# microsoft/UniSpeech

Hardware: NVIDIA H100
Metric: audio-sec/sec fwd+bwd (higher is better)
Workload: dtype bf16

## Files before the change

unispeech_b200/csrc/gemm.cu:

```cuda
#include <stdarg.h>
#include <stdlib.h>

#include <algorithm>
#include <mutex>

#include "../../include/unispeech_b200.h"
#include "common.h"
#include "gemm.cuh"

namespace b200 {

long long g_launch_count = 0;
static thread_local char g_err[512] = "";
char* last_error_buf() { return g_err; }
void set_last_error(const char* fmt, ...) {
  va_list ap;
  va_start(ap, fmt);
  vsnprintf(g_err, sizeof(g_err), fmt, ap);
  va_end(ap);
}
bool pdl_enabled() {
  static int v = -1;
  if (v < 0) {
    const char* e = getenv("B200S_PDL");
// ... 162 lines not shown

static int gemm_rows_impl(const void* a, long long a_bs, long long a_rs, int rows, int batches, int K, const void* w, int N,
                          void* out, long long out_bs, long long out_ld, const b200s_epilogue* epi, const int* m_valid,
                          b200s_stream stream) {
  B200_CHECK_ARG(a && w && out, "gemm_rows: null pointer");
  B200_CHECK_ARG(rows > 0 && batches > 0 && K > 0 && N > 0, "gemm_rows: bad sizes");
  B200_CHECK_ARG(K % 64 == 0, "gemm_rows: K=%d must be a multiple of 64", K);
  B200_CHECK_ARG(N % 8 == 0, "gemm_rows: N=%d must be a multiple of 8", N);
  if (check_epilogue(epi)) return -1;
  cudaStream_t st = static_cast<cudaStream_t>(stream);

  CUtensorMap ta, tb;
  ViewSpec va{a, {K, rows, batches, 1}, {a_rs, batches > 1 ? a_bs : 0, 0}, {64, 128, 1, 1}};
  if (batches == 1) va.strides[1] = 0;
  if (make_tmap(&ta, va)) return -3;

  GemmParams p;
  memset(&p, 0, sizeof(p));
  fill_epilogue(p, epi);
  p.out = {out, out_bs, out_ld};
  p.m_rows = rows;
  p.m_tile_stride = 128;
  p.m_tile_valid = 128;
  p.m_tiles_per_batch = ceil_div(rows, 128);
  p.m_tiles = p.m_tiles_per_batch * batches;
  p.n_total = N;
  p.k_blocks = K / 64;
  p.m_valid = m_valid;

  if (N >= 256 && m_valid == nullptr) {
    ViewSpec vb{w, {K, N, 1, 1}, {K, 0, 0}, {64, 256, 1, 1}};
    if (make_tmap(&tb, vb)) return -3;
    static std::once_flag once;
    static cudaError_t attr_err = cudaSuccess;
    std::call_once(once, [] {
      attr_err = cudaFuncSetAttribute(gemm_ws_kernel, cudaFuncAttributeMaxDynamicSharedMemorySize, WsCfg::kSmemBytes);
    });
    B200_CHECK_CUDA(attr_err);
    const int tiles = p.m_tiles * ceil_div(N, 256);
    B200_CHECK_CUDA(launch_pdl(gemm_ws_kernel, dim3(std::min(tiles, sm_count())), dim3(WsCfg::kThreads), WsCfg::kSmemBytes, st,
                               ta, tb, p));
    B200_CHECK_LAUNCH();
    return 0;
  }

  const int block_n = (N >= 128) ? 128 : 64;
  ViewSpec vb{w, {K, N, 1, 1}, {K, 0, 0}, {64, block_n, 1, 1}};
  if (make_tmap(&tb, vb)) return -3;

  p.n_out_stride = block_n;
  p.n_tile_valid = block_n;
  p.k_blocks_per_batch = 0;
  p.k_blocks_per_split = p.k_blocks;
  p.ca[0][4] = 1; p.ca[1][1] = 1; p.ca[2][2] = 1;
  p.cb[0][4] = 1; p.cb[1][3] = block_n;
  dim3 grid(ceil_div(N, block_n), p.m_tiles_per_batch * batches, 1);
  B200_CHECK_ARG(grid.y <= 65535, "gemm_rows: too many M tiles (%u)", grid.y);
  return block_n == 128 ? launch_gemm<128, false, false>(ta, tb, p, grid, st)
                        : launch_gemm<64, false, false>(ta, tb, p, grid, st);
}

int b200s_reserve_sms(int sms) {
  B200_CHECK_ARG(sms >= 0 && sms < sm_count(), "reserve_sms: %d out of range", sms);
  return 0;
}

int b200s_gemm_rows(const void* a, long long a_bs, long long a_rs, int rows, int batches, int K, const void* w, int N,
                    void* out, long long out_bs, long long out_ld, const b200s_epilogue* epi, b200s_stream stream) {
  return gemm_rows_impl(a, a_bs, a_rs, rows, batches, K, w, N, out, out_bs, out_ld, epi, nullptr, stream);
}

int b200s_gemm_rows_ragged(const void* a, long long a_bs, long long a_rs, int rows, int batches, int K, const void* w, int N,
                           void* out, long long out_bs, long long out_ld, const b200s_epilogue* epi, const int* m_valid,
                           b200s_stream stream) {
  return gemm_rows_impl(a, a_bs, a_rs, rows, batches, K, w, N, out, out_bs, out_ld, epi, m_valid, stream);
}

static int gemm_wgrad_impl(const void* y, long long y_bs, long long y_rs, const void* x, long long x_bs, long long x_rs,
                           int rows, int batches, int N, int K, float* dw, long long dw_ld, const int* k_valid,
                           b200s_stream stream) {
  B200_CHECK_ARG(y && x && dw, "gemm_wgrad: null pointer");
  B200_CHECK_ARG(rows > 0 && batches > 0 && K > 0 && N > 0, "gemm_wgrad: bad sizes");
  B200_CHECK_ARG(N % 8 == 0 && K % 8 == 0, "gemm_wgrad: N=%d, K=%d must be multiples of 8", N, K);
  const int block_n = (K >= 128) ? 128 : 64;

  CUtensorMap ta, tb;
  ViewSpec va{y, {N, rows, batches, 1}, {y_rs, batches > 1 ? y_bs : 0, 0}, {64, 64, 1, 1}};
  if (make_tmap(&ta, va)) return -3;
  ViewSpec vb{x, {K, rows, batches, 1}, {x_rs, batches > 1 ? x_bs : 0, 0}, {64, 64, 1, 1}};
  if (make_tmap(&tb, vb)) return -3;

  GemmParams p;
  memset(&p, 0, sizeof(p));
  p.m_rows = N;
  p.m_tile_stride = 128;
  p.m_tile_valid = 128;
  p.m_tiles_per_batch = ceil_div(N, 128);
  p.n_total = K;
  p.n_out_stride = block_n;
  p.n_tile_valid = block_n;
  p.k_blocks_per_batch = ceil_div(rows, 64);
  p.k_blocks = p.k_blocks_per_batch * batches;
  const int tiles = p.m_tiles_per_batch * ceil_div(K, block_n);
  int splits = ceil_div(2 * sm_count(), tiles);
  if (splits > p.k_blocks) splits = p.k_blocks;
  if (splits < 1) splits = 1;
  p.k_blocks_per_split = ceil_div(p.k_blocks, splits);
  splits = ceil_div(p.k_blocks, p.k_blocks_per_split);
  p.ca[0][1] = 1; p.ca[0][7] = 1; p.ca[1][4] = 1; p.ca[2][5] = 1;
  p.cb[0][3] = block_n; p.cb[0][7] = 1; p.cb[1][4] = 1; p.cb[2][5] = 1;
  p.flags = EPI_OUT_F32 | EPI_ATOMIC;
  fill_epilogue(p, nullptr);
  p.out = {dw, 0, dw_ld};
  p.k_valid = k_valid;
  dim3 grid(ceil_div(K, block_n), p.m_tiles_per_batch, splits);
  cudaStream_t st = static_cast<cudaStream_t>(stream);
  return block_n == 128 ? launch_gemm<128, true, true>(ta, tb, p, grid, st)
                        : launch_gemm<64, true, true>(ta, tb, p, grid, st);
}

int b200s_gemm_wgrad(const void* y, long long y_bs, long long y_rs, const void* x, long long x_bs, long long x_rs,
                     int rows, int batches, int N, int K, float* dw, long long dw_ld, b200s_stream stream) {
  return gemm_wgrad_impl(y, y_bs, y_rs, x, x_bs, x_rs, rows, batches, N, K, dw, dw_ld, nullptr, stream);
}

int b200s_gemm_wgrad_ragged(const void* y, long long y_bs, long long y_rs, const void* x, long long x_bs, long long x_rs,
                            int rows, int batches, int N, int K, float* dw, long long dw_ld, const int* k_valid,
                            b200s_stream stream) {
  return gemm_wgrad_impl(y, y_bs, y_rs, x, x_bs, x_rs, rows, batches, N, K, dw, dw_ld, k_valid, stream);
}

int b200s_posconv_gemm(const void* xpad, long long xpad_bs, int T, int B, int D, int G, int taps, const void* wp,
                       void* out, long long out_bs, long long out_ld, const b200s_epilogue* epi,
                       b200s_stream stream) {
  B200_CHECK_ARG(xpad && wp && out, "posconv_gemm: null pointer");
  B200_CHECK_ARG(D % G == 0, "posconv_gemm: D %% G != 0");
  const int Cg = D / G;
  B200_CHECK_ARG(Cg <= 64 && Cg % 8 == 0, "posconv_gemm: channels per group %d must be <=64 and a multiple of 8", Cg);
  B200_CHECK_ARG(D % 8 == 0, "posconv_gemm: D must be a multiple of 8");
  B200_CHECK_ARG(taps >= 1, "posconv_gemm: taps=%d must be positive", taps);
  if (check_epilogue(epi)) return -1;

  CUtensorMap ta, tb;
  ViewSpec vb{wp, {taps * 64LL, G * 64LL, 1, 1}, {taps * 64LL, 0, 0}, {64, 64, 1, 1}};
  if (make_tmap(&tb, vb)) return -3;

  GemmParams p;
  memset(&p, 0, sizeof(p));
  p.m_rows = T;
  p.m_tile_stride = 128;
  p.m_tile_valid = 128;
  p.m_tiles_per_batch = ceil_div(T, 128);
  p.n_total = D;
  p.n_out_stride = Cg;
  p.n_tile_valid = Cg;
  p.k_blocks = taps;
  p.k_blocks_per_batch = 0;
  p.k_blocks_per_split = taps;
  p.flags = 0;
  fill_epilogue(p, epi);
  p.out = {out, out_bs, out_ld};
  dim3 grid(G, p.m_tiles_per_batch * B, 1);
  cudaStream_t st = static_cast<cudaStream_t>(stream);

  if (taps <= 129) {
    ViewSpec vw{xpad, {D, T + taps - 1, B, 1}, {D, B > 1 ? xpad_bs : 0, 0}, {64, 256, 1, 1}};
    if (make_tmap(&ta, vw)) return -3;
    static std::once_flag once;
    static cudaError_t attr_err = cudaSuccess;
    std::call_once(once, [] {
      attr_err = cudaFuncSetAttribute(posconv_window_kernel, cudaFuncAttributeMaxDynamicSharedMemorySize,
                                      PosconvCfg::kSmemBytes);
    });
    B200_CHECK_CUDA(attr_err);
    B200_CHECK_CUDA(launch_pdl(posconv_window_kernel, grid, dim3(PosconvCfg::kThreads), PosconvCfg::kSmemBytes, st, ta, tb, p,
                               taps, Cg));
    B200_CHECK_LAUNCH();
    return 0;
  }
  ViewSpec va{xpad, {D, taps, T, B}, {D, D, xpad_bs}, {64, 1, 128, 1}};
  if (make_tmap(&ta, va)) return -3;
  p.ca[0][3] = Cg; p.ca[1][6] = 1; p.ca[2][1] = 1; p.ca[3][2] = 1;
  p.cb[0][4] = 1; p.cb[1][3] = 64;
  return launch_gemm<64, false, false>(ta, tb, p, grid, st);
}

int b200s_posconv_wgrad(const void* dy, long long dy_bs, long long dy_rs, const void* xpad, long long xpad_bs, int T,
                        int B, int D, int G, int taps, float* dwp, b200s_stream stream) {
  B200_CHECK_ARG(dy && xpad && dwp, "posconv_wgrad: null pointer");
  B200_CHECK_ARG(D % G == 0, "posconv_wgrad: D %% G != 0");
  const int Cg = D / G;
  B200_CHECK_ARG(Cg <= 64 && Cg % 8 == 0, "posconv_wgrad: channels per group %d must be <=64 and a multiple of 8", Cg);

  CUtensorMap ta, tb;
  ViewSpec va{dy, {D, T, B, 1}, {dy_rs, B > 1 ? dy_bs : 0, 0}, {64, 64, 1, 1}};
  if (make_tmap(&ta, va)) return -3;
  ViewSpec vb{xpad, {D, taps, T, B}, {D, D, xpad_bs}, {64, 1, 64, 1}};
  if (make_tmap(&tb, vb)) return -3;

  GemmParams p;
  memset(&p, 0, sizeof(p));
// ... 21 lines not shown
```

unispeech_b200/csrc/gemm.cuh:

```cuda
#pragma once
#include "ptx.cuh"

namespace b200 {

struct EpiTensor {
  void* p;
  long long bs;
  long long ld;
};

enum : int {
  EPI_GELU = 1,
  EPI_DGELU = 2,
  EPI_OUT_F32 = 4,
  EPI_ATOMIC = 8,
  EPI_COLSUM = 16,
  EPI_ACCUM = 32,
  EPI_GELU_STORE_GRAD = 64,
  EPI_AUX_IS_GRAD = 128,
};

constexpr int kCoordVars = 8;

struct GemmParams {
// ... 51 lines not shown
  e.out_bf = static_cast<__nv_bfloat16*>(p.out.p) + mb * p.out.bs + row * p.out.ld;
  e.out_f32 = static_cast<float*>(p.out.p) + mb * p.out.bs + row * p.out.ld;
  e.out2 = p.out2.p ? static_cast<__nv_bfloat16*>(p.out2.p) + mb * p.out2.bs + row * p.out2.ld : nullptr;
  e.aux = p.aux.p ? static_cast<const __nv_bfloat16*>(p.aux.p) + mb * p.aux.bs + row * p.aux.ld : nullptr;
  e.res1 = p.res1.p ? static_cast<const __nv_bfloat16*>(p.res1.p) + mb * p.res1.bs + row * p.res1.ld : nullptr;
  e.res2 = p.res2.p ? static_cast<const __nv_bfloat16*>(p.res2.p) + mb * p.res2.bs + row * p.res2.ld : nullptr;
  return e;
}
__device__ __forceinline__ void add_bf16x8(float* a8, const __nv_bfloat16* src) {
  const uint4 w = *reinterpret_cast<const uint4*>(src);
  const uint32_t wu[4] = {w.x, w.y, w.z, w.w};
#pragma unroll
  for (int j = 0; j < 4; ++j) {
    const float2 f = unpack_bf16x2(wu[j]);
    a8[2 * j] += f.x;
    a8[2 * j + 1] += f.y;
  }
}
__device__ __forceinline__ uint4 pack_bf16x8(const float* a8) {
  uint4 w;
  w.x = pack_bf16x2(a8[0], a8[1]); w.y = pack_bf16x2(a8[2], a8[3]);
  w.z = pack_bf16x2(a8[4], a8[5]); w.w = pack_bf16x2(a8[6], a8[7]);
  return w;
}

__device__ __forceinline__ void epilogue_chunk32(const GemmParams& p, const EpiRow& e, const float* src, int c0, int n_valid,
                                                 int col_base, bool row_ok, int lane) {
  const int flags = p.flags;
  float acc[32];
#pragma unroll
  for (int j = 0; j < 8; ++j) {
    const float4 v = reinterpret_cast<const float4*>(src)[j];
    acc[4 * j] = v.x; acc[4 * j + 1] = v.y; acc[4 * j + 2] = v.z; acc[4 * j + 3] = v.w;
  }
  const bool full = (c0 + 32 <= n_valid);
  if (p.bias != nullptr) {
    const float* bp = p.bias + col_base + c0;
    if (full) {
#pragma unroll
      for (int j = 0; j < 8; ++j) {
        const float4 b4 = __ldg(reinterpret_cast<const float4*>(bp) + j);
        acc[4 * j] += b4.x; acc[4 * j + 1] += b4.y; acc[4 * j + 2] += b4.z; acc[4 * j + 3] += b4.w;
      }
    } else {
#pragma unroll
      for (int j = 0; j < 32; ++j)
        if (c0 + j < n_valid) acc[j] += __ldg(bp + j);
    }
  }
  if (row_ok) {
    const int col0 = col_base + c0;
#pragma unroll
    for (int g = 0; g < 4; ++g) {
      if (!full && (c0 + g * 8 >= n_valid)) break;
      const int col = col0 + g * 8;
      float* a8 = acc + g * 8;
      if (flags & EPI_GELU) {
        if (flags & EPI_GELU_STORE_GRAD) {
          float g8[8];
#pragma unroll
          for (int j = 0; j < 8; ++j) a8[j] = gelu_with_grad_f(a8[j], g8[j]);
          if (e.out2 != nullptr) *reinterpret_cast<uint4*>(e.out2 + col) = pack_bf16x8(g8);
        } else {
          if (e.out2 != nullptr) *reinterpret_cast<uint4*>(e.out2 + col) = pack_bf16x8(a8);
#pragma unroll
          for (int j = 0; j < 8; ++j) a8[j] = gelu_f(a8[j]);
        }
      }
      if (flags & EPI_DGELU) {
        const uint4 w = *reinterpret_cast<const uint4*>(e.aux + col);
        const uint32_t wu[4] = {w.x, w.y, w.z, w.w};
#pragma unroll
        for (int j = 0; j < 4; ++j) {
          const float2 f = unpack_bf16x2(wu[j]);
          a8[2 * j] *= (flags & EPI_AUX_IS_GRAD) ? f.x : gelu_grad_f(f.x);
          a8[2 * j + 1] *= (flags & EPI_AUX_IS_GRAD) ? f.y : gelu_grad_f(f.y);
        }
      }
      if (e.res1 != nullptr) add_bf16x8(a8, e.res1 + col);
      if (e.res2 != nullptr) add_bf16x8(a8, e.res2 + col);
      if (flags & EPI_OUT_F32) {
        float* o = e.out_f32 + col;
        if (flags & EPI_ATOMIC) {
          asm volatile("red.global.add.v4.f32 [%0], {%1, %2, %3, %4};" ::"l"(o), "f"(a8[0]), "f"(a8[1]), "f"(a8[2]), "f"(a8[3])
                       : "memory");
          asm volatile("red.global.add.v4.f32 [%0], {%1, %2, %3, %4};" ::"l"(o + 4), "f"(a8[4]), "f"(a8[5]), "f"(a8[6]),
                       "f"(a8[7])
                       : "memory");
        } else if (flags & EPI_ACCUM) {
          float4 o0 = *reinterpret_cast<float4*>(o), o1 = *reinterpret_cast<float4*>(o + 4);
          o0.x += a8[0]; o0.y += a8[1]; o0.z += a8[2]; o0.w += a8[3];
          o1.x += a8[4]; o1.y += a8[5]; o1.z += a8[6]; o1.w += a8[7];
          *reinterpret_cast<float4*>(o) = o0;
          *reinterpret_cast<float4*>(o + 4) = o1;
        } else {
          *reinterpret_cast<float4*>(o) = make_float4(a8[0], a8[1], a8[2], a8[3]);
          *reinterpret_cast<float4*>(o + 4) = make_float4(a8[4], a8[5], a8[6], a8[7]);
        }
      } else {
        *reinterpret_cast<uint4*>(e.out_bf + col) = pack_bf16x8(a8);
      }
    }
  }
  if (flags & EPI_COLSUM) {
    float cv[32];
#pragma unroll
    for (int j = 0; j < 32; ++j) {
      float t = row_ok ? acc[j] : 0.0f;
      if (!(flags & EPI_OUT_F32)) t = __bfloat162float(__float2bfloat16_rn(t));
      cv[j] = t;
    }
    const float csum = warp_colsum32(cv, lane);
    if ((c0 + lane) < n_valid) atomicAdd(p.colsum + col_base + c0 + lane, csum);
  }
}


template <int N, bool TA, bool TB>
__device__ __forceinline__ void wgmma_tile(float* acc, uint64_t da, uint64_t db, uint32_t scale_d) {
  if constexpr (N == 64) wgmma_m64n64k16<TA ? 1 : 0, TB ? 1 : 0>(acc, da, db, scale_d);
  else wgmma_m64n128k16<TA ? 1 : 0, TB ? 1 : 0>(acc, da, db, scale_d);
}

template <int BLOCK_N>
__device__ __forceinline__ void gemm_consumer_tail(const GemmParams& p, const float* acc, float* acc_s, int mb, int m0,
                                                   int col_base, int n_valid, int m_valid) {
  constexpr int kPitch = BLOCK_N + 8;
  const int ew = threadIdx.x >> 5, lane = threadIdx.x & 31;
  named_bar_sync(1, 256);
  acc_to_smem<BLOCK_N>(acc, acc_s, kPitch, 64 * (ew >> 2));
  named_bar_sync(1, 256);
  const int r = (ew & 3) * 32 + lane;
  const EpiRow erow = make_epi_row(p, mb, static_cast<long long>(m0) + r);
#pragma unroll 1
  for (int c0 = (ew >> 2) * (BLOCK_N / 2); c0 < ((ew >> 2) + 1) * (BLOCK_N / 2); c0 += 32) {
    if (c0 >= n_valid) break;
    epilogue_chunk32(p, erow, acc_s + r * kPitch + c0, c0, n_valid, col_base, r < m_valid, lane);
  }
}

__device__ __forceinline__ void zero_dead_tile(const GemmParams& p, int mb, int m0, int col_base, int n_valid) {
  const int rows = min(p.m_tile_valid, p.m_rows - m0), c8 = n_valid / 8;
  for (int i = threadIdx.x; i < rows * c8; i += blockDim.x) {
    const long long row = static_cast<long long>(m0) + i / c8;
    const int col = col_base + (i % c8) * 8;
    *reinterpret_cast<uint4*>(static_cast<__nv_bfloat16*>(p.out.p) + mb * p.out.bs + row * p.out.ld + col) = make_uint4(0u, 0u, 0u, 0u);
    if (p.out2.p != nullptr)
      *reinterpret_cast<uint4*>(static_cast<__nv_bfloat16*>(p.out2.p) + mb * p.out2.bs + row * p.out2.ld + col) = make_uint4(0u, 0u, 0u, 0u);
  }
}

template <int BLOCK_N, bool A_MN, bool B_MN>
__global__ void __launch_bounds__(288, 2) gemm_bf16_kernel(const __grid_constant__ CUtensorMap tmA,
                                                           const __grid_constant__ CUtensorMap tmB,
                                                           const __grid_constant__ GemmParams p) {
  pdl_launch_dependents();
  using Cfg = GemmCfg<BLOCK_N>;
  constexpr int kStages = Cfg::kStages;

  const int warp = threadIdx.x >> 5;
  const int lane = threadIdx.x & 31;
  const int n_tile = blockIdx.x;
  const int mb = blockIdx.y / p.m_tiles_per_batch;
  const int m0 = (blockIdx.y % p.m_tiles_per_batch) * p.m_tile_stride;
  const int kb_begin = blockIdx.z * p.k_blocks_per_split;
  const int kb_end = min(kb_begin + p.k_blocks_per_split, p.k_blocks);
  if (kb_begin >= kb_end) return;
  const int col_base = n_tile * p.n_out_stride;
  const int n_valid = min(p.n_tile_valid, p.n_total - col_base);

  extern __shared__ uint8_t smem_raw[];
// ... 42 lines not shown
          v[5] = 0;
          v[4] = kb * 64;
        }
        v[6] = kb;
        uint8_t* sa = smem + s * Cfg::kStageBytes;
        uint8_t* sb = sa + Cfg::kABytes;
        mbar_expect_tx(&full_bar[s], Cfg::kStageBytes);
        if constexpr (!A_MN) {
          v[7] = 0;
          tma_load_4d(sa, &tmA, &full_bar[s], coord_dot(p.ca[0], v), coord_dot(p.ca[1], v), coord_dot(p.ca[2], v),
                      coord_dot(p.ca[3], v));
        } else {
#pragma unroll
          for (int i = 0; i < 2; ++i) {
            v[7] = 64 * i;
            tma_load_4d(sa + i * 8192, &tmA, &full_bar[s], coord_dot(p.ca[0], v), coord_dot(p.ca[1], v),
                        coord_dot(p.ca[2], v), coord_dot(p.ca[3], v));
          }
        }
        if constexpr (!B_MN) {
          v[7] = 0;
          tma_load_4d(sb, &tmB, &full_bar[s], coord_dot(p.cb[0], v), coord_dot(p.cb[1], v), coord_dot(p.cb[2], v),
                      coord_dot(p.cb[3], v));
        } else {
#pragma unroll
          for (int i = 0; i < BLOCK_N / 64; ++i) {
            v[7] = 64 * i;
            tma_load_4d(sb + i * 8192, &tmB, &full_bar[s], coord_dot(p.cb[0], v), coord_dot(p.cb[1], v),
                        coord_dot(p.cb[2], v), coord_dot(p.cb[3], v));
          }
        }
      }
    }
  } else {
    const int c = warp >> 2;
    float acc[BLOCK_N / 2];
    int it = 0;
    for (int kb = kb_begin; kb < kb_end; ++kb) {
      if (!kb_live(kb)) continue;
      const int s = it % kStages;
      mbar_wait(&full_bar[s], (it / kStages) & 1);
      const uint32_t sa = smem_u32(smem + s * Cfg::kStageBytes) + c * 8192;
      const uint32_t sb = smem_u32(smem + s * Cfg::kStageBytes + Cfg::kABytes);
      wgmma_fence();
#pragma unroll
      for (int k = 0; k < 4; ++k) {
        const uint64_t da = A_MN ? make_smem_desc_sw128(sa + k * 2048, 8192, 1024) : make_smem_desc_sw128(sa + k * 32, 16, 1024);
        const uint64_t db = B_MN ? make_smem_desc_sw128(sb + k * 2048, 8192, 1024) : make_smem_desc_sw128(sb + k * 32, 16, 1024);
        wgmma_tile<BLOCK_N, A_MN, B_MN>(acc, da, db, (it > 0 || k > 0) ? 1u : 0u);
      }
      wgmma_commit();
      wgmma_wait<1>();
      if (it > 0 && lane == 0) mbar_arrive(&empty_bar[(it - 1) % kStages]);
      ++it;
    }
    wgmma_wait<0>();
    if (it == 0) {
#pragma unroll
      for (int i = 0; i < BLOCK_N / 2; ++i) acc[i] = 0.f;
    }
    gemm_consumer_tail<BLOCK_N>(p, acc, reinterpret_cast<float*>(smem), mb, m0, col_base, n_valid,
                                min(p.m_tile_valid, p.m_rows - m0));
  }
}

struct WsCfg {
  static constexpr int kStages = 3;
  static constexpr int kABytes = 128 * 128;
  static constexpr int kBBytes = 256 * 128;
  static constexpr int kStageBytes = kABytes + kBBytes;
  static constexpr int kEpiBytes = 64 * 64 * 4;
  static constexpr int kPfBytes = 3 * 8 * 128 * 8;
  static constexpr int kSmemBytes = kStages * kStageBytes + 2 * kEpiBytes + 2 * kPfBytes + 1024;
  static constexpr int kThreads = 384;
  static_assert(kSmemBytes + 1024 <= 232448, "one CTA per SM");
};

__device__ __forceinline__ void add_bf16x4(float* v, uint2 w) {
  const float2 f0 = unpack_bf16x2(w.x), f1 = unpack_bf16x2(w.y);
  v[0] += f0.x; v[1] += f0.y; v[2] += f1.x; v[3] += f1.y;
}
__device__ __forceinline__ uint2 pack_bf16x4(const float* v) { return make_uint2(pack_bf16x2(v[0], v[1]), pack_bf16x2(v[2], v[3])); }

__global__ void __launch_bounds__(384, 1) gemm_ws_kernel(const __grid_constant__ CUtensorMap tmA,
                                                         const __grid_constant__ CUtensorMap tmB,
                                                         const __grid_constant__ GemmParams p) {
  pdl_launch_dependents();
  using Cfg = WsCfg;
  constexpr int kStages = Cfg::kStages;
  const int wg = threadIdx.x >> 7;
  const int lane = threadIdx.x & 31;
  const int n_tiles = (p.n_total + 255) / 256;
  const int num_tiles = p.m_tiles * n_tiles;

  extern __shared__ uint8_t smem_raw[];
  uint8_t* smem = smem_raw + ((1024u - (smem_u32(smem_raw) & 1023u)) & 1023u);
  __shared__ uint64_t full_bar[kStages];
  __shared__ uint64_t empty_bar[kStages];

  if (threadIdx.x == 0) {
    tma_prefetch_desc(&tmA);
    tma_prefetch_desc(&tmB);
#pragma unroll
    for (int s = 0; s < kStages; ++s) {
      mbar_init(&full_bar[s], 1);
      mbar_init(&empty_bar[s], 8);
    }
    fence_mbar_init();
  }
  __syncthreads();
  pdl_wait();

  if (wg == 0) {
    setmaxnreg_dec<40>();
    if (threadIdx.x == 0) {
      int it = 0;
      for (int tile = blockIdx.x; tile < num_tiles; tile += gridDim.x) {
        const int mt = tile / n_tiles, n_tile = tile - mt * n_tiles;
        const int mb = mt / p.m_tiles_per_batch, m0 = (mt - mb * p.m_tiles_per_batch) * 128;
        for (int kb = 0; kb < p.k_blocks; ++kb, ++it) {
          const int s = it % kStages;
          mbar_wait(&empty_bar[s], ((it / kStages) & 1) ^ 1);
          uint8_t* sa = smem + s * Cfg::kStageBytes;
          mbar_expect_tx(&full_bar[s], Cfg::kStageBytes);
          tma_load_4d(sa, &tmA, &full_bar[s], kb * 64, m0, mb, 0);
          tma_load_4d(sa + Cfg::kABytes, &tmB, &full_bar[s], kb * 64, n_tile * 256, 0, 0);
        }
      }
    }
    return;
  }

  setmaxnreg_inc<232>();
  const int c = wg - 1;
  const int t = threadIdx.x & 127, w = t >> 5;
  float* stage = reinterpret_cast<float*>(smem + kStages * Cfg::kStageBytes + c * Cfg::kEpiBytes);
  uint2* pf = reinterpret_cast<uint2*>(smem + kStages * Cfg::kStageBytes + 2 * Cfg::kEpiBytes + c * Cfg::kPfBytes);
  const int cq = 4 * (lane & 15);
  const EpiTensor* const pf_src[3] = {&p.aux, &p.res1, &p.res2};
  float acc[128];
  int it = 0;
  for (int tile = blockIdx.x; tile < p.m_tiles * n_tiles; tile += gridDim.x) {
    const int mt = tile / n_tiles, n_tile = tile - mt * n_tiles;
    const int mb = mt / p.m_tiles_per_batch, m0 = (mt - mb * p.m_tiles_per_batch) * 128;
    const int col_base = n_tile * 256;
    const int n_valid = min(256, p.n_total - col_base);
    const int rows_here = min(128, p.m_rows - m0) - 64 * c;
    auto prefetch = [&](int j) {
      const int cl = 64 * j + cq;
      if (cl < n_valid) {
#pragma unroll
        for (int q = 0; q < 3; ++q) {
          const EpiTensor& e = *pf_src[q];
          if (e.p == nullptr) continue;
#pragma unroll
          for (int i = 0; i < 8; ++i) {
            const int r = 16 * w + 2 * i + (lane >> 4);
            if (r < rows_here)
              cp_async_8(pf + (q * 8 + i) * 128 + t, static_cast<const __nv_bfloat16*>(e.p) + mb * e.bs +
                                                         (static_cast<long long>(m0) + 64 * c + r) * e.ld + col_base + cl);
          }
        }
      }
      cp_async_commit();
    };
    prefetch(0);
    for (int kb = 0; kb < p.k_blocks; ++kb, ++it) {
      const int s = it % kStages;
      mbar_wait(&full_bar[s], (it / kStages) & 1);
      const uint32_t sa = smem_u32(smem + s * Cfg::kStageBytes) + c * 8192;
      const uint32_t sb = smem_u32(smem + s * Cfg::kStageBytes + Cfg::kABytes);
      wgmma_fence();
#pragma unroll
      for (int k = 0; k < 4; ++k)
        wgmma_m64n256k16<0, 0>(acc, make_smem_desc_sw128(sa + k * 32, 16, 1024), make_smem_desc_sw128(sb + k * 32, 16, 1024),
                               (kb > 0 || k > 0) ? 1u : 0u);
      wgmma_commit();
      wgmma_wait<1>();
      if (kb > 0 && lane == 0) mbar_arrive(&empty_bar[(it - 1) % kStages]);
    }
    wgmma_wait<0>();
    if (lane == 0) mbar_arrive(&empty_bar[(it - 1) % kStages]);

    const int flags = p.flags;
#pragma unroll
    for (int j = 0; j < 4; ++j) {
      if (64 * j >= n_valid) break;
      named_bar_sync(1 + c, 128);
#pragma unroll
      for (int i = 32 * j; i < 32 * j + 32; i += 2) {
        const int r = 16 * w + (lane >> 2) + 8 * ((i >> 1) & 1);
        const int cc = 8 * ((i >> 2) - 8 * j) + 2 * (lane & 3);
        *reinterpret_cast<float2*>(stage + r * 64 + (cc ^ ((r & 3) << 3))) = make_float2(acc[i], acc[i + 1]);
      }
      const int cl = 64 * j + cq;
      const bool col_ok = cl < n_valid;
      const int col = col_base + cl;
      named_bar_sync(1 + c, 128);
      float4 b4 = make_float4(0.f, 0.f, 0.f, 0.f);
      if (p.bias != nullptr && col_ok) b4 = __ldg(reinterpret_cast<const float4*>(p.bias + col));
      float cs[4] = {0.f, 0.f, 0.f, 0.f};
      cp_async_wait_all();
#pragma unroll 4
      for (int i = 0; i < 8; ++i) {
        const int r = 16 * w + 2 * i + (lane >> 4);
        const float4 v4 = *reinterpret_cast<const float4*>(stage + r * 64 + (cq ^ ((r & 3) << 3)));
        if (!col_ok || r >= rows_here) continue;
        float v[4] = {v4.x + b4.x, v4.y + b4.y, v4.z + b4.z, v4.w + b4.w};
        const long long row = static_cast<long long>(m0) + 64 * c + r;
        if (flags & EPI_GELU) {
          __nv_bfloat16* o2 =
              p.out2.p ? static_cast<__nv_bfloat16*>(p.out2.p) + mb * p.out2.bs + row * p.out2.ld + col : nullptr;
          if (flags & EPI_GELU_STORE_GRAD) {
            float g[4];
#pragma unroll
            for (int k = 0; k < 4; ++k) v[k] = gelu_with_grad_f(v[k], g[k]);
            if (o2 != nullptr) *reinterpret_cast<uint2*>(o2) = pack_bf16x4(g);
          } else {
            if (o2 != nullptr) *reinterpret_cast<uint2*>(o2) = pack_bf16x4(v);
#pragma unroll
            for (int k = 0; k < 4; ++k) v[k] = gelu_f(v[k]);
          }
        }
        if (flags & EPI_DGELU) {
          const uint2 a = pf[(0 * 8 + i) * 128 + t];
          const float2 f0 = unpack_bf16x2(a.x), f1 = unpack_bf16x2(a.y);
          const float f[4] = {f0.x, f0.y, f1.x, f1.y};
#pragma unroll
          for (int k = 0; k < 4; ++k) v[k] *= (flags & EPI_AUX_IS_GRAD) ? f[k] : gelu_grad_f(f[k]);
        }
        if (p.res1.p != nullptr) add_bf16x4(v, pf[(1 * 8 + i) * 128 + t]);
        if (p.res2.p != nullptr) add_bf16x4(v, pf[(2 * 8 + i) * 128 + t]);
        *reinterpret_cast<uint2*>(static_cast<__nv_bfloat16*>(p.out.p) + mb * p.out.bs + row * p.out.ld + col) = pack_bf16x4(v);
        if (flags & EPI_COLSUM) {
#pragma unroll
          for (int k = 0; k < 4; ++k) cs[k] += __bfloat162float(__float2bfloat16_rn(v[k]));
        }
      }
      if (j < 3) prefetch(j + 1);
      if (flags & EPI_COLSUM) {
#pragma unroll
        for (int k = 0; k < 4; ++k) cs[k] += __shfl_xor_sync(0xffffffffu, cs[k], 16);
        named_bar_sync(1 + c, 128);
        if (lane < 16) *reinterpret_cast<float4*>(stage + w * 64 + cq) = make_float4(cs[0], cs[1], cs[2], cs[3]);
        named_bar_sync(1 + c, 128);
        if (t < 64 && 64 * j + t < n_valid)
          atomicAdd(p.colsum + col_base + 64 * j + t, stage[t] + stage[64 + t] + stage[128 + t] + stage[192 + t]);
      }
    }
  }
}

struct PosconvCfg {
  static constexpr int kStages = 6;
  static constexpr int kABytes = 256 * 128;
  static constexpr int kBBytes = 64 * 128;
  static constexpr int kSmemBytes = kABytes + kStages * kBBytes + 1024;
  static constexpr int kThreads = 288;
};

__global__ void __launch_bounds__(288, 2) posconv_window_kernel(const __grid_constant__ CUtensorMap tmA,
                                                                const __grid_constant__ CUtensorMap tmB,
                                                                const __grid_constant__ GemmParams p, int taps, int cg) {
  pdl_launch_dependents();
  using Cfg = PosconvCfg;
  constexpr int kStages = Cfg::kStages;
  const int warp = threadIdx.x >> 5;
  const int lane = threadIdx.x & 31;
  const int g = blockIdx.x;
  const int mb = blockIdx.y / p.m_tiles_per_batch;
  const int m0 = (blockIdx.y % p.m_tiles_per_batch) * 128;

  extern __shared__ uint8_t smem_raw[];
  uint8_t* smem = smem_raw + ((1024u - (smem_u32(smem_raw) & 1023u)) & 1023u);
  uint8_t* sA = smem;
  uint8_t* sB = smem + Cfg::kABytes;
  __shared__ uint64_t a_full, full_bar[kStages], empty_bar[kStages];

  if (threadIdx.x == 0) {
    tma_prefetch_desc(&tmA);
    tma_prefetch_desc(&tmB);
    mbar_init(&a_full, 1);
#pragma unroll
    for (int s = 0; s < kStages; ++s) {
      mbar_init(&full_bar[s], 1);
      mbar_init(&empty_bar[s], 8);
    }
    fence_mbar_init();
  }
  __syncthreads();
  pdl_wait();

  if (warp == 8) {
    if (lane == 0) {
      mbar_expect_tx(&a_full, Cfg::kABytes);
      tma_load_4d(sA, &tmA, &a_full, g * cg, m0, mb, 0);
      for (int j = 0; j < taps; ++j) {
        const int s = j % kStages;
        mbar_wait(&empty_bar[s], ((j / kStages) & 1) ^ 1);
        mbar_expect_tx(&full_bar[s], Cfg::kBBytes);
        tma_load_4d(sB + s * Cfg::kBBytes, &tmB, &full_bar[s], j * 64, g * 64, 0, 0);
      }
    }
  } else {
    const int c = warp >> 2;
    float acc[32];
    mbar_wait(&a_full, 0);
    for (int j = 0; j < taps; ++j) {
      const int s = j % kStages;
      mbar_wait(&full_bar[s], (j / kStages) & 1);
      const uint32_t sa = smem_u32(sA) + (64 * c + j) * 128;
      const uint32_t sb = smem_u32(sB + s * Cfg::kBBytes);
      wgmma_fence();
#pragma unroll
      for (int k = 0; k < 4; ++k)
        wgmma_tile<64, false, false>(acc, make_smem_desc_sw128(sa + k * 32, 16, 1024), make_smem_desc_sw128(sb + k * 32, 16, 1024),
                                     (j > 0 || k > 0) ? 1u : 0u);
      wgmma_commit();
      wgmma_wait<1>();
      if (j > 0 && lane == 0) mbar_arrive(&empty_bar[(j - 1) % kStages]);
    }
    wgmma_wait<0>();
    gemm_consumer_tail<64>(p, acc, reinterpret_cast<float*>(smem), mb, m0, g * cg, cg, min(128, p.m_rows - m0));
  }
}

}
```

unispeech_b200/csrc/ptx.cuh:

```cuda
#pragma once
#include <cuda.h>
#include <cuda_bf16.h>
#include <cuda_runtime.h>
#include <stdint.h>

namespace b200 {

__device__ __forceinline__ uint32_t smem_u32(const void* p) {
  return static_cast<uint32_t>(__cvta_generic_to_shared(p));
}

__device__ __forceinline__ void pdl_launch_dependents() { asm volatile("griddepcontrol.launch_dependents;" ::: "memory"); }
__device__ __forceinline__ void pdl_wait() { asm volatile("griddepcontrol.wait;" ::: "memory"); }
__device__ __forceinline__ void pdl_grid_sync() {
  pdl_launch_dependents();
  pdl_wait();
}

__device__ __forceinline__ void mbar_init(uint64_t* bar, uint32_t count) {
  asm volatile("mbarrier.init.shared::cta.b64 [%0], %1;" ::"r"(smem_u32(bar)), "r"(count) : "memory");
}
__device__ __forceinline__ void fence_mbar_init() {
  asm volatile("fence.mbarrier_init.release.cluster;" ::: "memory");
}
__device__ __forceinline__ void mbar_expect_tx(uint64_t* bar, uint32_t bytes) {
  asm volatile("mbarrier.arrive.expect_tx.shared::cta.b64 _, [%0], %1;" ::"r"(smem_u32(bar)), "r"(bytes) : "memory");
}
__device__ __forceinline__ void mbar_arrive(uint64_t* bar) {
  asm volatile("mbarrier.arrive.shared::cta.b64 _, [%0];" ::"r"(smem_u32(bar)) : "memory");
}
__device__ __forceinline__ bool mbar_try_wait(uint64_t* bar, uint32_t parity) {
  uint32_t done;
  asm volatile(
      "{\n\t.reg .pred p;\n\t"
      "mbarrier.try_wait.parity.shared::cta.b64 p, [%1], %2;\n\t"
      "selp.u32 %0, 1, 0, p;\n\t}"
      : "=r"(done)
      : "r"(smem_u32(bar)), "r"(parity)
      : "memory");
  return done != 0;
}
__device__ __forceinline__ void mbar_wait(uint64_t* bar, uint32_t parity) {
  uint32_t spins = 0;
  while (!mbar_try_wait(bar, parity)) {
    if (++spins > (1u << 28)) __trap();
  }
}

__device__ __forceinline__ void fence_proxy_async_smem() {
  asm volatile("fence.proxy.async.shared::cta;" ::: "memory");
}
__device__ __forceinline__ void named_bar_sync(int id, int count) {
  asm volatile("bar.sync %0, %1;" ::"r"(id), "r"(count) : "memory");
}

__device__ __forceinline__ void tma_prefetch_desc(const CUtensorMap* m) {
  asm volatile("prefetch.tensormap [%0];" ::"l"(reinterpret_cast<uint64_t>(m)) : "memory");
}
__device__ __forceinline__ void tma_load_2d(void* dst, const CUtensorMap* m, uint64_t* bar, int c0, int c1) {
  asm volatile(
      "cp.async.bulk.tensor.2d.shared::cluster.global.mbarrier::complete_tx::bytes [%0], [%1, {%3, %4}], [%2];" ::"r"(
          smem_u32(dst)),
      "l"(reinterpret_cast<uint64_t>(m)), "r"(smem_u32(bar)), "r"(c0), "r"(c1)
      : "memory");
}
__device__ __forceinline__ void tma_load_3d(void* dst, const CUtensorMap* m, uint64_t* bar, int c0, int c1, int c2) {
  asm volatile(
      "cp.async.bulk.tensor.3d.shared::cluster.global.mbarrier::complete_tx::bytes [%0], [%1, {%3, %4, %5}], [%2];" ::"r"(
          smem_u32(dst)),
      "l"(reinterpret_cast<uint64_t>(m)), "r"(smem_u32(bar)), "r"(c0), "r"(c1), "r"(c2)
      : "memory");
}
__device__ __forceinline__ void tma_load_4d(void* dst, const CUtensorMap* m, uint64_t* bar, int c0, int c1, int c2,
                                            int c3) {
  asm volatile(
      "cp.async.bulk.tensor.4d.shared::cluster.global.mbarrier::complete_tx::bytes [%0], [%1, {%3, %4, %5, %6}], "
      "[%2];" ::"r"(smem_u32(dst)),
      "l"(reinterpret_cast<uint64_t>(m)), "r"(smem_u32(bar)), "r"(c0), "r"(c1), "r"(c2), "r"(c3)
      : "memory");
}

__device__ __forceinline__ void tma_store_4d(const CUtensorMap* m, uint32_t smem_src, int c0, int c1, int c2, int c3) {
  asm volatile("cp.async.bulk.tensor.4d.global.shared::cta.bulk_group [%0, {%2, %3, %4, %5}], [%1];" ::"l"(
                   reinterpret_cast<uint64_t>(m)),
               "r"(smem_src), "r"(c0), "r"(c1), "r"(c2), "r"(c3)
               : "memory");
}
__device__ __forceinline__ void bulk_commit() { asm volatile("cp.async.bulk.commit_group;" ::: "memory"); }
__device__ __forceinline__ void bulk_wait_read0() { asm volatile("cp.async.bulk.wait_group.read 0;" ::: "memory"); }
__device__ __forceinline__ void bulk_wait0() { asm volatile("cp.async.bulk.wait_group 0;" ::: "memory"); }

__device__ __forceinline__ void cp_async_8(void* smem_dst, const void* gsrc) {
  asm volatile("cp.async.ca.shared.global [%0], [%1], 8;" ::"r"(smem_u32(smem_dst)), "l"(gsrc) : "memory");
}
__device__ __forceinline__ void cp_async_commit() { asm volatile("cp.async.commit_group;" ::: "memory"); }
__device__ __forceinline__ void cp_async_wait_all() { asm volatile("cp.async.wait_group 0;" ::: "memory"); }

__device__ __forceinline__ uint64_t make_smem_desc_sw128(uint32_t smem_addr, uint32_t lbo_bytes, uint32_t sbo_bytes) {
  uint64_t d = 0;
  d |= static_cast<uint64_t>((smem_addr >> 4) & 0x3FFF);
  d |= static_cast<uint64_t>((lbo_bytes >> 4) & 0x3FFF) << 16;
  d |= static_cast<uint64_t>((sbo_bytes >> 4) & 0x3FFF) << 32;
  d |= static_cast<uint64_t>(1) << 62;
  return d;
}
__device__ __forceinline__ void wgmma_fence() { asm volatile("wgmma.fence.sync.aligned;" ::: "memory"); }
__device__ __forceinline__ void wgmma_commit() { asm volatile("wgmma.commit_group.sync.aligned;" ::: "memory"); }
template <int N>
__device__ __forceinline__ void wgmma_wait() {
  asm volatile("wgmma.wait_group.sync.aligned %0;" ::"n"(N) : "memory");
}
template <int TA, int TB>
__device__ __forceinline__ void wgmma_m64n64k16(float* d, uint64_t desc_a, uint64_t desc_b, uint32_t scale_d) {
  asm volatile(
      "{\n\t.reg .pred p;\n\t"
      "setp.ne.b32 p, %34, 0;\n\t"
      "wgmma.mma_async.sync.aligned.m64n64k16.f32.bf16.bf16 "
      "{%0, %1, %2, %3, %4, %5, %6, %7, %8, %9, %10, %11, %12, %13, %14, %15, %16, %17, %18, %19, %20, %21, %22, %23, %24, %25, %26, %27, %28, %29, %30, %31}, "
      "%32, %33, p, 1, 1, %35, %36;\n\t}"
      : "+f"(d[0]), "+f"(d[1]), "+f"(d[2]), "+f"(d[3]), "+f"(d[4]), "+f"(d[5]), "+f"(d[6]), "+f"(d[7]), "+f"(d[8]), "+f"(d[9]), "+f"(d[10]), "+f"(d[11]), "+f"(d[12]), "+f"(d[13]), "+f"(d[14]), "+f"(d[15]), "+f"(d[16]), "+f"(d[17]), "+f"(d[18]), "+f"(d[19]), "+f"(d[20]), "+f"(d[21]), "+f"(d[22]), "+f"(d[23]), "+f"(d[24]), "+f"(d[25]), "+f"(d[26]), "+f"(d[27]), "+f"(d[28]), "+f"(d[29]), "+f"(d[30]), "+f"(d[31])
      : "l"(desc_a), "l"(desc_b), "r"(scale_d), "n"(TA), "n"(TB)
      : "memory");
}

template <int TA, int TB>
__device__ __forceinline__ void wgmma_m64n128k16(float* d, uint64_t desc_a, uint64_t desc_b, uint32_t scale_d) {
  asm volatile(
      "{\n\t.reg .pred p;\n\t"
      "setp.ne.b32 p, %66, 0;\n\t"
      "wgmma.mma_async.sync.aligned.m64n128k16.f32.bf16.bf16 "
      "{%0, %1, %2, %3, %4, %5, %6, %7, %8, %9, %10, %11, %12, %13, %14, %15, %16, %17, %18, %19, %20, %21, %22, %23, %24, %25, %26, %27, %28, %29, %30, %31, %32, %33, %34, %35, %36, %37, %38, %39, %40, %41, %42, %43, %44, %45, %46, %47, %48, %49, %50, %51, %52, %53, %54, %55, %56, %57, %58, %59, %60, %61, %62, %63}, "
      "%64, %65, p, 1, 1, %67, %68;\n\t}"
      : "+f"(d[0]), "+f"(d[1]), "+f"(d[2]), "+f"(d[3]), "+f"(d[4]), "+f"(d[5]), "+f"(d[6]), "+f"(d[7]), "+f"(d[8]), "+f"(d[9]), "+f"(d[10]), "+f"(d[11]), "+f"(d[12]), "+f"(d[13]), "+f"(d[14]), "+f"(d[15]), "+f"(d[16]), "+f"(d[17]), "+f"(d[18]), "+f"(d[19]), "+f"(d[20]), "+f"(d[21]), "+f"(d[22]), "+f"(d[23]), "+f"(d[24]), "+f"(d[25]), "+f"(d[26]), "+f"(d[27]), "+f"(d[28]), "+f"(d[29]), "+f"(d[30]), "+f"(d[31]), "+f"(d[32]), "+f"(d[33]), "+f"(d[34]), "+f"(d[35]), "+f"(d[36]), "+f"(d[37]), "+f"(d[38]), "+f"(d[39]), "+f"(d[40]), "+f"(d[41]), "+f"(d[42]), "+f"(d[43]), "+f"(d[44]), "+f"(d[45]), "+f"(d[46]), "+f"(d[47]), "+f"(d[48]), "+f"(d[49]), "+f"(d[50]), "+f"(d[51]), "+f"(d[52]), "+f"(d[53]), "+f"(d[54]), "+f"(d[55]), "+f"(d[56]), "+f"(d[57]), "+f"(d[58]), "+f"(d[59]), "+f"(d[60]), "+f"(d[61]), "+f"(d[62]), "+f"(d[63])
      : "l"(desc_a), "l"(desc_b), "r"(scale_d), "n"(TA), "n"(TB)
      : "memory");
}

template <int TA, int TB>
__device__ __forceinline__ void wgmma_m64n256k16(float* d, uint64_t desc_a, uint64_t desc_b, uint32_t scale_d) {
  asm volatile(
      "{\n\t.reg .pred p;\n\t"
      "setp.ne.b32 p, %130, 0;\n\t"
      "wgmma.mma_async.sync.aligned.m64n256k16.f32.bf16.bf16 "
      "{%0, %1, %2, %3, %4, %5, %6, %7, %8, %9, %10, %11, %12, %13, %14, %15, %16, %17, %18, %19, %20, %21, %22, %23, %24, %25, %26, %27, %28, %29, %30, %31, %32, %33, %34, %35, %36, %37, %38, %39, %40, %41, %42, %43, %44, %45, %46, %47, %48, %49, %50, %51, %52, %53, %54, %55, %56, %57, %58, %59, %60, %61, %62, %63, %64, %65, %66, %67, %68, %69, %70, %71, %72, %73, %74, %75, %76, %77, %78, %79, %80, %81, %82, %83, %84, %85, %86, %87, %88, %89, %90, %91, %92, %93, %94, %95, %96, %97, %98, %99, %100, %101, %102, %103, %104, %105, %106, %107, %108, %109, %110, %111, %112, %113, %114, %115, %116, %117, %118, %119, %120, %121, %122, %123, %124, %125, %126, %127}, "
      "%128, %129, p, 1, 1, %131, %132;\n\t}"
      : "+f"(d[0]), "+f"(d[1]), "+f"(d[2]), "+f"(d[3]), "+f"(d[4]), "+f"(d[5]), "+f"(d[6]), "+f"(d[7]), "+f"(d[8]), "+f"(d[9]), "+f"(d[10]), "+f"(d[11]), "+f"(d[12]), "+f"(d[13]), "+f"(d[14]), "+f"(d[15]), "+f"(d[16]), "+f"(d[17]), "+f"(d[18]), "+f"(d[19]), "+f"(d[20]), "+f"(d[21]), "+f"(d[22]), "+f"(d[23]), "+f"(d[24]), "+f"(d[25]), "+f"(d[26]), "+f"(d[27]), "+f"(d[28]), "+f"(d[29]), "+f"(d[30]), "+f"(d[31]), "+f"(d[32]), "+f"(d[33]), "+f"(d[34]), "+f"(d[35]), "+f"(d[36]), "+f"(d[37]), "+f"(d[38]), "+f"(d[39]), "+f"(d[40]), "+f"(d[41]), "+f"(d[42]), "+f"(d[43]), "+f"(d[44]), "+f"(d[45]), "+f"(d[46]), "+f"(d[47]), "+f"(d[48]), "+f"(d[49]), "+f"(d[50]), "+f"(d[51]), "+f"(d[52]), "+f"(d[53]), "+f"(d[54]), "+f"(d[55]), "+f"(d[56]), "+f"(d[57]), "+f"(d[58]), "+f"(d[59]), "+f"(d[60]), "+f"(d[61]), "+f"(d[62]), "+f"(d[63]), "+f"(d[64]), "+f"(d[65]), "+f"(d[66]), "+f"(d[67]), "+f"(d[68]), "+f"(d[69]), "+f"(d[70]), "+f"(d[71]), "+f"(d[72]), "+f"(d[73]), "+f"(d[74]), "+f"(d[75]), "+f"(d[76]), "+f"(d[77]), "+f"(d[78]), "+f"(d[79]), "+f"(d[80]), "+f"(d[81]), "+f"(d[82]), "+f"(d[83]), "+f"(d[84]), "+f"(d[85]), "+f"(d[86]), "+f"(d[87]), "+f"(d[88]), "+f"(d[89]), "+f"(d[90]), "+f"(d[91]), "+f"(d[92]), "+f"(d[93]), "+f"(d[94]), "+f"(d[95]), "+f"(d[96]), "+f"(d[97]), "+f"(d[98]), "+f"(d[99]), "+f"(d[100]), "+f"(d[101]), "+f"(d[102]), "+f"(d[103]), "+f"(d[104]), "+f"(d[105]), "+f"(d[106]), "+f"(d[107]), "+f"(d[108]), "+f"(d[109]), "+f"(d[110]), "+f"(d[111]), "+f"(d[112]), "+f"(d[113]), "+f"(d[114]), "+f"(d[115]), "+f"(d[116]), "+f"(d[117]), "+f"(d[118]), "+f"(d[119]), "+f"(d[120]), "+f"(d[121]), "+f"(d[122]), "+f"(d[123]), "+f"(d[124]), "+f"(d[125]), "+f"(d[126]), "+f"(d[127])
      : "l"(desc_a), "l"(desc_b), "r"(scale_d), "n"(TA), "n"(TB)
      : "memory");
}

template <int N>
__device__ __forceinline__ void setmaxnreg_dec() {
  asm volatile("setmaxnreg.dec.sync.aligned.u32 %0;" ::"n"(N));
}
template <int N>
__device__ __forceinline__ void setmaxnreg_inc() {
  asm volatile("setmaxnreg.inc.sync.aligned.u32 %0;" ::"n"(N));
}

template <int N>
__device__ __forceinline__ void acc_to_smem(const float* d, float* tile, int pitch, int row0) {
  const int t = threadIdx.x & 127, w = t >> 5, l = t & 31;
  float* base = tile + (row0 + 16 * w + (l >> 2)) * pitch + 2 * (l & 3);
#pragma unroll
  for (int i = 0; i < N / 2; i += 2)
    *reinterpret_cast<float2*>(base + 8 * ((i >> 1) & 1) * pitch + 8 * (i >> 2)) = make_float2(d[i], d[i + 1]);
}
template <int N>
__device__ __forceinline__ void smem_to_acc(float* d, const float* tile, int pitch, int row0) {
  const int t = threadIdx.x & 127, w = t >> 5, l = t & 31;
  const float* base = tile + (row0 + 16 * w + (l >> 2)) * pitch + 2 * (l & 3);
#pragma unroll
  for (int i = 0; i < N / 2; i += 2) {
    const float2 v = *reinterpret_cast<const float2*>(base + 8 * ((i >> 1) & 1) * pitch + 8 * (i >> 2));
    d[i] = v.x;
    d[i + 1] = v.y;
  }
}

// ... 140 lines not shown
```

Measured before the change: 2209.

## Add warp-specialized stream-K weight-gradient GEMM kernel for wide K

For K >= 256 the weight-gradient GEMM now runs a new persistent warp-specialized kernel that uses 128x256 tiles with m64n256 wgmma. It splits the flattened (tile, k-block) work evenly across one CTA per SM, stream-K style, and accumulates fp32 partials with vector red.add atomics staged through swizzled shared memory. The aim is higher tensor-core utilization and balanced load compared with the split-K 128/64-wide generic kernel. The cost is more atomic traffic at piece boundaries and extra complexity in index bookkeeping for ragged k_valid batches. The fallback path now always uses block_n 64.

```diff
diff --git a/unispeech_b200/csrc/gemm.cu b/unispeech_b200/csrc/gemm.cu
--- a/unispeech_b200/csrc/gemm.cu
+++ b/unispeech_b200/csrc/gemm.cu
@@ -268,7 +268,7 @@
   B200_CHECK_ARG(y && x && dw, "gemm_wgrad: null pointer");
   B200_CHECK_ARG(rows > 0 && batches > 0 && K > 0 && N > 0, "gemm_wgrad: bad sizes");
   B200_CHECK_ARG(N % 8 == 0 && K % 8 == 0, "gemm_wgrad: N=%d, K=%d must be multiples of 8", N, K);
-  const int block_n = (K >= 128) ? 128 : 64;
+  cudaStream_t st = static_cast<cudaStream_t>(stream);
 
   CUtensorMap ta, tb;
   ViewSpec va{y, {N, rows, batches, 1}, {y_rs, batches > 1 ? y_bs : 0, 0}, {64, 64, 1, 1}};
@@ -283,10 +283,31 @@
   p.m_tile_valid = 128;
   p.m_tiles_per_batch = ceil_div(N, 128);
   p.n_total = K;
+  p.k_blocks_per_batch = ceil_div(rows, 64);
+  p.k_blocks = p.k_blocks_per_batch * batches;
+  p.flags = EPI_OUT_F32 | EPI_ATOMIC;
+  fill_epilogue(p, nullptr);
+  p.out = {dw, 0, dw_ld};
+  p.k_valid = k_valid;
+
+  if (K >= 256) {
+    p.m_tiles = p.m_tiles_per_batch;
+    static std::once_flag once;
+    static cudaError_t attr_err = cudaSuccess;
+    std::call_once(once, [] {
+      attr_err = cudaFuncSetAttribute(gemm_ws_wgrad_kernel, cudaFuncAttributeMaxDynamicSharedMemorySize, WsCfg::kSmemBytes);
+    });
+    B200_CHECK_CUDA(attr_err);
+    const long long work = static_cast<long long>(p.m_tiles) * ceil_div(K, 256) * p.k_blocks;
+    B200_CHECK_CUDA(launch_pdl(gemm_ws_wgrad_kernel, dim3(static_cast<unsigned>(std::min<long long>(work, sm_count()))),
+                               dim3(WsCfg::kThreads), WsCfg::kSmemBytes, st, ta, tb, p));
+    B200_CHECK_LAUNCH();
+    return 0;
+  }
+
+  const int block_n = 64;
   p.n_out_stride = block_n;
   p.n_tile_valid = block_n;
-  p.k_blocks_per_batch = ceil_div(rows, 64);
-  p.k_blocks = p.k_blocks_per_batch * batches;
   const int tiles = p.m_tiles_per_batch * ceil_div(K, block_n);
   int splits = ceil_div(2 * sm_count(), tiles);
   if (splits > p.k_blocks) splits = p.k_blocks;
@@ -295,14 +316,8 @@
   splits = ceil_div(p.k_blocks, p.k_blocks_per_split);
   p.ca[0][1] = 1; p.ca[0][7] = 1; p.ca[1][4] = 1; p.ca[2][5] = 1;
   p.cb[0][3] = block_n; p.cb[0][7] = 1; p.cb[1][4] = 1; p.cb[2][5] = 1;
-  p.flags = EPI_OUT_F32 | EPI_ATOMIC;
-  fill_epilogue(p, nullptr);
-  p.out = {dw, 0, dw_ld};
-  p.k_valid = k_valid;
   dim3 grid(ceil_div(K, block_n), p.m_tiles_per_batch, splits);
-  cudaStream_t st = static_cast<cudaStream_t>(stream);
-  return block_n == 128 ? launch_gemm<128, true, true>(ta, tb, p, grid, st)
-                        : launch_gemm<64, true, true>(ta, tb, p, grid, st);
+  return launch_gemm<64, true, true>(ta, tb, p, grid, st);
 }
 
 int b200s_gemm_wgrad(const void* y, long long y_bs, long long y_rs, const void* x, long long x_bs, long long x_rs,
diff --git a/unispeech_b200/csrc/gemm.cuh b/unispeech_b200/csrc/gemm.cuh
--- a/unispeech_b200/csrc/gemm.cuh
+++ b/unispeech_b200/csrc/gemm.cuh
@@ -157,11 +157,8 @@
       if (flags & EPI_OUT_F32) {
         float* o = e.out_f32 + col;
         if (flags & EPI_ATOMIC) {
-          asm volatile("red.global.add.v4.f32 [%0], {%1, %2, %3, %4};" ::"l"(o), "f"(a8[0]), "f"(a8[1]), "f"(a8[2]), "f"(a8[3])
-                       : "memory");
-          asm volatile("red.global.add.v4.f32 [%0], {%1, %2, %3, %4};" ::"l"(o + 4), "f"(a8[4]), "f"(a8[5]), "f"(a8[6]),
-                       "f"(a8[7])
-                       : "memory");
+          red_add_f32x4(o, a8[0], a8[1], a8[2], a8[3]);
+          red_add_f32x4(o + 4, a8[4], a8[5], a8[6], a8[7]);
         } else if (flags & EPI_ACCUM) {
           float4 o0 = *reinterpret_cast<float4*>(o), o1 = *reinterpret_cast<float4*>(o + 4);
           o0.x += a8[0]; o0.y += a8[1]; o0.z += a8[2]; o0.w += a8[3];
@@ -370,6 +367,20 @@
 }
 __device__ __forceinline__ uint2 pack_bf16x4(const float* v) { return make_uint2(pack_bf16x2(v[0], v[1]), pack_bf16x2(v[2], v[3])); }
 
+__device__ __forceinline__ void ws_stage_chunk(const float* acc, float* stage, int j, int w, int lane) {
+#pragma unroll
+  for (int i = 32 * j; i < 32 * j + 32; i += 2) {
+    const int r = 16 * w + (lane >> 2) + 8 * ((i >> 1) & 1);
+    const int cc = 8 * ((i >> 2) - 8 * j) + 2 * (lane & 3);
+    *reinterpret_cast<float2*>(stage + r * 64 + (cc ^ ((r & 3) << 3))) = make_float2(acc[i], acc[i + 1]);
+  }
+}
+__device__ __forceinline__ int ws_lane_col(int lane) { return 4 * (lane & 15); }
+__device__ __forceinline__ int ws_chunk_row(int w, int i, int lane) { return 16 * w + 2 * i + (lane >> 4); }
+__device__ __forceinline__ float4 ws_load_row(const float* stage, int r, int cq) {
+  return *reinterpret_cast<const float4*>(stage + r * 64 + (cq ^ ((r & 3) << 3)));
+}
+
 __global__ void __launch_bounds__(384, 1) gemm_ws_kernel(const __grid_constant__ CUtensorMap tmA,
                                                          const __grid_constant__ CUtensorMap tmB,
                                                          const __grid_constant__ GemmParams p) {
@@ -424,7 +435,7 @@
   const int t = threadIdx.x & 127, w = t >> 5;
   float* stage = reinterpret_cast<float*>(smem + kStages * Cfg::kStageBytes + c * Cfg::kEpiBytes);
   uint2* pf = reinterpret_cast<uint2*>(smem + kStages * Cfg::kStageBytes + 2 * Cfg::kEpiBytes + c * Cfg::kPfBytes);
-  const int cq = 4 * (lane & 15);
+  const int cq = ws_lane_col(lane);
   const EpiTensor* const pf_src[3] = {&p.aux, &p.res1, &p.res2};
   float acc[128];
   int it = 0;
@@ -443,7 +454,7 @@
           if (e.p == nullptr) continue;
 #pragma unroll
           for (int i = 0; i < 8; ++i) {
-            const int r = 16 * w + 2 * i + (lane >> 4);
+            const int r = ws_chunk_row(w, i, lane);
             if (r < rows_here)
               cp_async_8(pf + (q * 8 + i) * 128 + t, static_cast<const __nv_bfloat16*>(e.p) + mb * e.bs +
                                                          (static_cast<long long>(m0) + 64 * c + r) * e.ld + col_base + cl);
@@ -475,12 +486,7 @@
     for (int j = 0; j < 4; ++j) {
       if (64 * j >= n_valid) break;
       named_bar_sync(1 + c, 128);
-#pragma unroll
-      for (int i = 32 * j; i < 32 * j + 32; i += 2) {
-        const int r = 16 * w + (lane >> 2) + 8 * ((i >> 1) & 1);
-        const int cc = 8 * ((i >> 2) - 8 * j) + 2 * (lane & 3);
-        *reinterpret_cast<float2*>(stage + r * 64 + (cc ^ ((r & 3) << 3))) = make_float2(acc[i], acc[i + 1]);
-      }
+      ws_stage_chunk(acc, stage, j, w, lane);
       const int cl = 64 * j + cq;
       const bool col_ok = cl < n_valid;
       const int col = col_base + cl;
@@ -491,8 +497,8 @@
       cp_async_wait_all();
 #pragma unroll 4
       for (int i = 0; i < 8; ++i) {
-        const int r = 16 * w + 2 * i + (lane >> 4);
-        const float4 v4 = *reinterpret_cast<const float4*>(stage + r * 64 + (cq ^ ((r & 3) << 3)));
+        const int r = ws_chunk_row(w, i, lane);
+        const float4 v4 = ws_load_row(stage, r, cq);
         if (!col_ok || r >= rows_here) continue;
         float v[4] = {v4.x + b4.x, v4.y + b4.y, v4.z + b4.z, v4.w + b4.w};
         const long long row = static_cast<long long>(m0) + 64 * c + r;
@@ -534,6 +540,140 @@
         named_bar_sync(1 + c, 128);
         if (t < 64 && 64 * j + t < n_valid)
           atomicAdd(p.colsum + col_base + 64 * j + t, stage[t] + stage[64 + t] + stage[128 + t] + stage[192 + t]);
+      }
+    }
+  }
+}
+
+__device__ __forceinline__ int wgrad_live_blocks(const GemmParams& p, int b) {
+  return p.k_valid == nullptr ? p.k_blocks_per_batch : min(p.k_blocks_per_batch, (max(__ldg(p.k_valid + b), 0) + 63) / 64);
+}
+
+__global__ void __launch_bounds__(384, 1) gemm_ws_wgrad_kernel(const __grid_constant__ CUtensorMap tmA,
+                                                               const __grid_constant__ CUtensorMap tmB,
+                                                               const __grid_constant__ GemmParams p) {
+  pdl_launch_dependents();
+  using Cfg = WsCfg;
+  constexpr int kStages = Cfg::kStages;
+  const int wg = threadIdx.x >> 7;
+  const int lane = threadIdx.x & 31;
+  const int n_tiles = (p.n_total + 255) / 256;
+
+  extern __shared__ uint8_t smem_raw[];
+  uint8_t* smem = smem_raw + ((1024u - (smem_u32(smem_raw) & 1023u)) & 1023u);
+  __shared__ uint64_t full_bar[kStages];
+  __shared__ uint64_t empty_bar[kStages];
+
+  if (threadIdx.x == 0) {
+    tma_prefetch_desc(&tmA);
+    tma_prefetch_desc(&tmB);
+#pragma unroll
+    for (int s = 0; s < kStages; ++s) {
+      mbar_init(&full_bar[s], 1);
+      mbar_init(&empty_bar[s], 8);
+    }
+    fence_mbar_init();
+  }
+  __syncthreads();
+  pdl_wait();
+
+  const int batches = p.k_blocks / p.k_blocks_per_batch;
+  int kl = 0;
+  for (int b = 0; b < batches; ++b) kl += wgrad_live_blocks(p, b);
+  const long long total = static_cast<long long>(p.m_tiles) * n_tiles * kl;
+  const long long g_begin = blockIdx.x * total / gridDim.x, g_end = (blockIdx.x + 1) * total / gridDim.x;
+  auto piece = [&](long long g, int& t, int& j0, int& j1) {
+    t = static_cast<int>(g / kl);
+    j0 = static_cast<int>(g - static_cast<long long>(t) * kl);
+    j1 = static_cast<int>(min(static_cast<long long>(kl), j0 + (g_end - g)));
+  };
+
+  if (wg == 0) {
+    setmaxnreg_dec<40>();
+    if (threadIdx.x == 0) {
+      int it = 0;
+      for (long long g = g_begin; g < g_end;) {
+        int t, j0, j1;
+        piece(g, t, j0, j1);
+        g += j1 - j0;
+        const int mt = t / n_tiles, n_tile = t - mt * n_tiles;
+        const long long x = static_cast<long long>(t) * kl;
+        const long long i0 = ((x + 1) * gridDim.x + total - 1) / total - 1;
+        int l = j0 + static_cast<int>((x - i0 * total / gridDim.x) % kl);
+        if (l >= kl) l -= kl;
+        int kbatch = 0;
+        while (l >= wgrad_live_blocks(p, kbatch)) l -= wgrad_live_blocks(p, kbatch++);
+        for (int j = j0; j < j1; ++j, ++it) {
+          const int s = it % kStages;
+          mbar_wait(&empty_bar[s], ((it / kStages) & 1) ^ 1);
+          uint8_t* sa = smem + s * Cfg::kStageBytes;
+          uint8_t* sb = sa + Cfg::kABytes;
+          mbar_expect_tx(&full_bar[s], Cfg::kStageBytes);
+#pragma unroll
+          for (int i = 0; i < 2; ++i) tma_load_4d(sa + i * 8192, &tmA, &full_bar[s], mt * 128 + 64 * i, l * 64, kbatch, 0);
+#pragma unroll
+          for (int i = 0; i < 4; ++i) tma_load_4d(sb + i * 8192, &tmB, &full_bar[s], n_tile * 256 + 64 * i, l * 64, kbatch, 0);
+          if (++l == wgrad_live_blocks(p, kbatch)) {
+            l = 0;
+            do {
+              if (++kbatch == batches) kbatch = 0;
+            } while (wgrad_live_blocks(p, kbatch) == 0);
+          }
+        }
+      }
+    }
+    return;
+  }
+
+  setmaxnreg_inc<232>();
+  const int c = wg - 1;
+  const int w = (threadIdx.x & 127) >> 5;
+  float* stage = reinterpret_cast<float*>(smem + kStages * Cfg::kStageBytes + c * Cfg::kEpiBytes);
+  const int cq = ws_lane_col(lane);
+  float acc[128];
+  int it = 0;
+  for (long long g = g_begin; g < g_end;) {
+    int t, j0, j1;
+    piece(g, t, j0, j1);
+    g += j1 - j0;
+    for (int j = 0; j < j1 - j0; ++j, ++it) {
+      const int s = it % kStages;
+      mbar_wait(&full_bar[s], (it / kStages) & 1);
+      const uint32_t sa = smem_u32(smem + s * Cfg::kStageBytes) + c * 8192;
+      const uint32_t sb = smem_u32(smem + s * Cfg::kStageBytes + Cfg::kABytes);
+      wgmma_fence();
+#pragma unroll
+      for (int k = 0; k < 4; ++k)
+        wgmma_m64n256k16<1, 1>(acc, make_smem_desc_sw128(sa + k * 2048, 8192, 1024),
+                               make_smem_desc_sw128(sb + k * 2048, 8192, 1024), (j > 0 || k > 0) ? 1u : 0u);
+      wgmma_commit();
+      wgmma_wait<1>();
+      if (j > 0 && lane == 0) mbar_arrive(&empty_bar[(it - 1) % kStages]);
+    }
+    wgmma_wait<0>();
+    if (lane == 0) mbar_arrive(&empty_bar[(it - 1) % kStages]);
+
+    const int mt = t / n_tiles, n_tile = t - mt * n_tiles;
+    const int m0 = mt * 128, col_base = n_tile * 256;
+    const int n_valid = min(256, p.n_total - col_base);
+    const int rows_here = min(128, p.m_rows - m0) - 64 * c;
+    float* out = static_cast<float*>(p.out.p) + (static_cast<long long>(m0) + 64 * c) * p.out.ld + col_base;
+#pragma unroll
+    for (int j = 0; j < 4; ++j) {
+      if (64 * j >= n_valid) break;
+      named_bar_sync(1 + c, 128);
+      ws_stage_chunk(acc, stage, j, w, lane);
+      named_bar_sync(1 + c, 128);
+      const int cl = 64 * j + cq;
+      if (cl < n_valid) {
+#pragma unroll
+        for (int i = 0; i < 8; ++i) {
+          const int r = ws_chunk_row(w, i, lane);
+          if (r < rows_here) {
+            const float4 v = ws_load_row(stage, r, cq);
+            red_add_f32x4(out + r * p.out.ld + cl, v.x, v.y, v.z, v.w);
+          }
+        }
       }
     }
   }
diff --git a/unispeech_b200/csrc/ptx.cuh b/unispeech_b200/csrc/ptx.cuh
--- a/unispeech_b200/csrc/ptx.cuh
+++ b/unispeech_b200/csrc/ptx.cuh
@@ -95,6 +95,10 @@
 }
 __device__ __forceinline__ void cp_async_commit() { asm volatile("cp.async.commit_group;" ::: "memory"); }
 __device__ __forceinline__ void cp_async_wait_all() { asm volatile("cp.async.wait_group 0;" ::: "memory"); }
+
+__device__ __forceinline__ void red_add_f32x4(float* p, float a, float b, float c, float d) {
+  asm volatile("red.global.add.v4.f32 [%0], {%1, %2, %3, %4};" ::"l"(p), "f"(a), "f"(b), "f"(c), "f"(d) : "memory");
+}
 
 __device__ __forceinline__ uint64_t make_smem_desc_sw128(uint32_t smem_addr, uint32_t lbo_bytes, uint32_t sbo_bytes) {
   uint64_t d = 0;
```

Result: faster. 2385 (median of 6 runs) (+7.9%).
